# lh3/ropebwt2

Measured on AMD Instinct MI355X. Metric: Gsymbols/s inserted (wall-clock), bit-identical .fmd, higher is better.
Workload: dtype u8; 1 GPU; configs[1]: 100000000 x 101 bp synthetic reads (splitmix64 seed 42), -bsR -m4g, 1 x MI355X; step = one -m batch (40844297/40844297/18311406 reads); 20 steps = 7 job(s) of 3 batches, each job on an empty index (the last job stops after batch 2); reads_per_job=100000000, symbols=69532236588, symbols_per_gpu=69532236588, parallelism=1 GPU, driver=single engine, counts_ok=True

## Files before the change

ropebwt2_amd/csrc/rb2_kernels.h:

```cpp
#pragma once
#include "rb2_device.h"

namespace rb2 {


__device__ __forceinline__ uint32_t zero_bytes(uint32_t x)
{
	const uint32_t t = ((x & 0x7f7f7f7fu) + 0x7f7f7f7fu) | x;
	return __popc(~t & 0x80808080u);
}

__device__ __forceinline__ void load64(const uint8_t *s, uint64_t len, uint64_t base, uint32_t w[16])
{
	if (base + 64 <= len) {
		const uint4 *p = (const uint4*)(s + base);
#pragma unroll
		for (int i = 0; i < 4; ++i) { uint4 v = p[i]; w[4*i] = v.x; w[4*i+1] = v.y; w[4*i+2] = v.z; w[4*i+3] = v.w; }
	} else {
#pragma unroll
		for (int i = 0; i < 16; ++i) {
			uint32_t x = 0;
			for (int k = 0; k < 4; ++k) {
				const uint64_t p = base + 4*i + k;
				x |= (uint32_t)(p < len ? s[p] : 0xffu) << (8*k);
// ... 1185 lines not shown
		const int v = min(GSYM, max(0, (int)nvalid - ln * GSYM));
		pl_acc(A, b0, b1, b2, bits_below((uint32_t)v));
		uint64_t *dst = (uint64_t*)newp.data + gl * LEAFW + ln;
		dst[0] = b0; dst[LEAFG] = b1; dst[2 * LEAFG] = b2;
	}
	const uint32_t r0 = wave_sum<uint32_t>(A.p0 | A.p1 << 16), r1 = wave_sum<uint32_t>(A.p2 | A.p01 << 16), r2 = wave_sum<uint32_t>(A.p02);
	if (ln == 0) {
		PlAcc T;
		T.p0 = r0 & 0xffffu; T.p1 = r0 >> 16; T.p2 = r1 & 0xffffu; T.p01 = r1 >> 16; T.p02 = r2;
		uint32_t c[6];
		pl_finish(T, nvalid, c);
		LeafMeta m;
		for (int sy = 0; sy < 6; ++sy) m.c[sy] = (uint16_t)c[sy];
		m.npre = 0; m.n = (uint16_t)nvalid;
		newp.own[gl] = m;
	}
	__builtin_amdgcn_fence(__ATOMIC_SEQ_CST, "wavefront"); __builtin_amdgcn_wave_barrier();
	}
}


__device__ __forceinline__ void split_body(Ctl *ctl, const PoolView &pool, const uint32_t *SPL, uint32_t spl_cap, uint32_t epoch , Mailbox *mb,
		const uint32_t bidx, const uint32_t nblk, uint16_t (*s_row)[7][SB], uint32_t round1)
{
	const uint32_t tid = threadIdx.x & 255u;
	if (bidx == 0 && tid == 0) mb->progress = round1;
	if (ctl->overflow) { if (bidx == 0 && tid == 0) mb->void_round = ctl->overflow; return; }
	const int wv = __builtin_amdgcn_readfirstlane(tid >> 6);
	const int ln = lane_id();
	const uint32_t nsp_raw = ctl->nsplit2[(round1 - 1u) & 1u];
	const uint32_t nsp_all = min(nsp_raw, spl_cap);
	if (nsp_raw > spl_cap && bidx == 0 && tid == 0) { ctl->sbfull = 1; mb->respread = 1; }
	for (uint32_t e = bidx * MW + wv; e < nsp_all; e += nblk * MW) {
		const uint64_t gl = SPL[e], sb = gl / SB;
		uint32_t mine = 0;
		if (ln == 0) mine = atomicExch((uint32_t*)dir_row(pool, sb, 7), epoch) != epoch;
		if (!__shfl((int)mine, 0)) continue;
		uint16_t v[7];
#pragma unroll
		for (int r = 0; r < 7; ++r) v[r] = ln < SB ? dir_row(pool, sb, r)[ln] : (uint16_t)0;
		const uint32_t used = (uint32_t)__popcll(__ballot(ln < SB && (v[0] & FILL_MASK) > 0));
		uint32_t marked = (uint32_t)__ballot(ln < SB && (v[0] & FILL_MASK) > (uint32_t)(LEAF - SP_MARGIN));
		if (marked == 0) continue;
		const uint32_t room = SB - used;
		if ((uint32_t)__popc(marked) > room) {
			if (ln == 0) { ctl->sbfull = 1; mb->respread = 1; }
			while ((uint32_t)__popc(marked) > room) marked &= ~(1u << (31 - __builtin_clz(marked)));
			if (marked == 0) continue;
		}
		const uint32_t first = (uint32_t)__builtin_ctz(marked);
		uint16_t (*R)[SB] = s_row[wv];
		if (ln < (int)used && !((marked >> ln) & 1u)) {
			const uint32_t nj = (uint32_t)ln + (uint32_t)__popc(marked & ((1u << ln) - 1u));
#pragma unroll
			for (int r = 0; r < 7; ++r) R[r][nj] = v[r];
		}
		uint64_t *leaves = (uint64_t*)pool.data + sb * SB * LEAFW;
		const bool wl = ln < LEAFW;
		const uint32_t gq = (uint32_t)(ln & 15);
		for (int c0 = SB - 8; c0 >= 0; c0 -= 8) {
		if ((uint32_t)(c0 + 8) <= first || (uint32_t)c0 >= used) continue;
		uint64_t W[8];
#pragma unroll
		for (int j = 0; j < 8; ++j) { const uint32_t k = (uint32_t)(c0 + j); W[j] = (wl && k >= first && k < used) ? leaves[(uint64_t)k * LEAFW + ln] : 0ull; }
#pragma unroll
		for (int j = 0; j < 8; ++j) {
			const int k = c0 + j;
			if ((uint32_t)k < first || (uint32_t)k >= used) continue;
			const uint32_t nk = (uint32_t)k + (uint32_t)__popc(marked & ((1u << k) - 1u));
			const uint64_t w = W[j];
			if (!((marked >> k) & 1u)) { if (nk != (uint32_t)k && wl) leaves[(uint64_t)nk * LEAFW + ln] = w; continue; }
			const uint32_t nraw = (uint32_t)__builtin_amdgcn_readlane((int)v[0], k), n = nraw & FILL_MASK, p2f = nraw & FILL_P2;
			uint32_t ck[6];
#pragma unroll
			for (int s = 0; s < 6; ++s) ck[s] = (uint32_t)__builtin_amdgcn_readlane((int)v[1 + s], k);
			const uint32_t hg = (n / 2) >> 6, h = hg << 6;
			const uint64_t w1 = (uint64_t)__shfl((unsigned long long)w, (ln + 16) & 63), w2 = (uint64_t)__shfl((unsigned long long)w, (ln + 32) & 63);
			PlAcc A;
			pl_acc(A, w, w1, leaf_p2(p2f != 0, w, w1, w2), (ln < LEAFG && gq < hg) ? ~0ull : 0ull);
			const uint32_t r0 = lane63(dpp_incl_add(A.p0 | A.p1 << 16)), r1 = lane63(dpp_incl_add(A.p2 | A.p01 << 16)), r2 = lane63(dpp_incl_add(A.p02));
			PlAcc T;
			T.p0 = r0 & 0xffffu; T.p1 = r0 >> 16; T.p2 = r1 & 0xffffu; T.p01 = r1 >> 16; T.p02 = r2;
			uint32_t c1[6];
			pl_finish(T, h, c1);
			const uint64_t up = (uint64_t)__shfl((unsigned long long)w, (ln + (int)hg) & 63);
			if (wl) {
				leaves[(uint64_t)(nk + 1) * LEAFW + ln] = gq + hg < (uint32_t)LEAFG ? up : 0ull;
				leaves[(uint64_t)nk * LEAFW + ln] = gq < hg ? w : 0ull;
			}
			if (ln == 0) {
				R[0][nk] = (uint16_t)(h | p2f); R[0][nk + 1] = (uint16_t)((n - h) | p2f);
#pragma unroll
				for (int s = 0; s < 6; ++s) { R[1 + s][nk] = (uint16_t)c1[s]; R[1 + s][nk + 1] = (uint16_t)(ck[s] - c1[s]); }
			}
		}
		}
		__builtin_amdgcn_fence(__ATOMIC_SEQ_CST, "wavefront"); __builtin_amdgcn_wave_barrier();
		const uint32_t nused = used + (uint32_t)__popc(marked);
		if (ln == 0) atomicAdd((unsigned long long*)&ctl->nsplit_total, (unsigned long long)__popc(marked));
		if ((uint32_t)ln >= first && (uint32_t)ln < nused) {
#pragma unroll
			for (int r = 0; r < 7; ++r) dir_row(pool, sb, r)[ln] = R[r][ln];
		}
		__builtin_amdgcn_fence(__ATOMIC_SEQ_CST, "wavefront"); __builtin_amdgcn_wave_barrier();
	}
}
__global__ __launch_bounds__(256) void k_split(Ctl *ctl, PoolView pool, const uint32_t *SPL, uint32_t spl_cap, uint32_t epoch, Mailbox *mb, SbBase *scan2, uint32_t round1)
{
	__shared__ uint16_t s_row[MW][7][SB];
	const uint32_t nb = gridDim.x - (scan2 ? 1u : 0u);
	if (scan2 && blockIdx.x == nb) { __shared__ uint64_t s_w2[4]; sbscan2_lean<256, 2>(ctl, scan2, s_w2); return; }
	split_body(ctl, pool, SPL, spl_cap, epoch, mb, blockIdx.x, nb, s_row, round1);
}

}
#include "rb2_merge.h"
namespace rb2 {


template <bool STRIDE> __global__ __launch_bounds__(256) void k_meta_sb(const Ctl *ctl, int nside, PoolView newp, SbTot *sbtot, int sparse)
{
	const int ln = lane_id();
	const uint64_t nsb = ctl->nsb_total;
	for (uint64_t sbw = ((uint64_t)blockIdx.x * 4 + wave_id()) * 2; sbw < nsb; sbw += (uint64_t)gridDim.x * 8) {
	const uint64_t sb = sbw + (ln >> 5);
	const bool live = sb < nsb;
	const uint64_t gl = sb * SB + (ln & 31);
	const uint64_t sb0 = ctl->rope[nside][ln < NR ? ln : NR - 1].sb0;
	const uint64_t sbA = sb - (ln >> 5);
	const int rA = max(0, (int)__popcll(__ballot(ln < NR && sb0 <= sbA)) - 1);
	const int rB = max(0, (int)__popcll(__ballot(ln < NR && sb0 <= sbA + 1)) - 1);
	const RopeDesc &rp = ctl->rope[nside][(ln >> 5) ? rB : rA];
	const bool ok = live && gl >= rp.leaf0 && gl < rp.leaf0 + rp.nleaves;
	LeafMeta m;
	for (int s = 0; s < 6; ++s) m.c[s] = 0;
	m.npre = 0; m.n = 0;
	if (ok) m = newp.own[gl];
	const uint32_t e01 = m.c[0] | (uint32_t)m.c[1] << 16, e23 = m.c[2] | (uint32_t)m.c[3] << 16, e45 = m.c[4] | (uint32_t)m.c[5] << 16;
	uint32_t s01 = dpp_incl_add(e01), s23 = dpp_incl_add(e23), s45 = dpp_incl_add(e45);
	const uint32_t h01 = (uint32_t)__builtin_amdgcn_readlane((int)s01, 31), h23 = (uint32_t)__builtin_amdgcn_readlane((int)s23, 31), h45 = (uint32_t)__builtin_amdgcn_readlane((int)s45, 31);
	if (ln >> 5) { s01 -= h01; s23 -= h23; s45 -= h45; }
	const uint32_t x01 = s01 - e01, x23 = s23 - e23, x45 = s45 - e45;
	if (sparse) {
		if (live) {
			uint16_t *dr = dir_row(newp, sb, 0) + (ln & 31);
			dr[0] = (uint16_t)(m.n | ((m.c[0] | m.c[5]) ? FILL_P2 : 0u));
#pragma unroll
			for (int s = 0; s < 6; ++s) dr[(1 + s) * SB] = m.c[s];
			dr[7 * SB] = 0;
		}
	} else if (ok) {
		m.c[0] = (uint16_t)x01; m.c[1] = (uint16_t)(x01 >> 16); m.c[2] = (uint16_t)x23; m.c[3] = (uint16_t)(x23 >> 16);
		m.c[4] = (uint16_t)x45; m.c[5] = (uint16_t)(x45 >> 16);
		m.npre = (uint16_t)((x01 & 0xffffu) + (x01 >> 16) + (x23 & 0xffffu) + (x23 >> 16) + (x45 & 0xffffu) + (x45 >> 16));
		newp.meta[gl] = m;
	}
	if ((ln & 31) == 31 && live) {
		SbTot c;
		c.p01 = s01; c.p23 = s23; c.p45 = s45; c.pad = 0;
		sbtot[sb] = c;
	}
	if (!STRIDE) return;
	}
}

constexpr int SBT = 4;
constexpr int SB2T = 512;
template <int NT, int CT = 8> __device__ __forceinline__ void sbscan2_body(const Ctl *ctl, SbBase *base, uint64_t (*s_w)[NT / 64])
{
	constexpr int SB2T = NT;
	const uint64_t nc = (ctl->nsb_total + SCHUNK - 1) / SCHUNK;
	const int ln = lane_id(), wv = __builtin_amdgcn_readfirstlane(threadIdx.x >> 6);
	uint64_t run[6] = {0, 0, 0, 0, 0, 0};
	for (uint64_t i0 = 0; i0 < nc; i0 += CT * SB2T) {
		const uint64_t j0 = i0 + (uint64_t)threadIdx.x * CT;
		uint64_t v[CT][6], tot[6] = {0, 0, 0, 0, 0, 0};
#pragma unroll
		for (int k = 0; k < CT; ++k)
#pragma unroll
			for (int s = 0; s < 6; ++s) v[k][s] = j0 + k < nc ? base[j0 + k].cum[s] : 0ull;
#pragma unroll
		for (int k = 0; k < CT; ++k)
#pragma unroll
			for (int s = 0; s < 6; ++s) { const uint64_t x = v[k][s]; v[k][s] = tot[s]; tot[s] += x; }
		uint64_t inc[6];
#pragma unroll
		for (int s = 0; s < 6; ++s) { inc[s] = wave_incl_add<uint64_t>(tot[s]); if (ln == 63) s_w[s][wv] = inc[s]; }
		__syncthreads();
		uint64_t b0[6];
#pragma unroll
		for (int s = 0; s < 6; ++s) {
			uint64_t off = 0, all = 0;
			for (int w = 0; w < SB2T / 64; ++w) { const uint64_t x = s_w[s][w]; if (w < wv) off += x; all += x; }
			b0[s] = run[s] + off + inc[s] - tot[s];
			run[s] += all;
		}
#pragma unroll
		for (int k = 0; k < CT; ++k) if (j0 + k < nc) {
			SbBase o;
#pragma unroll
			for (int s = 0; s < 6; ++s) o.cum[s] = b0[s] + v[k][s];
			o.pos = o.cum[0] + o.cum[1] + o.cum[2] + o.cum[3] + o.cum[4] + o.cum[5]; o.pad = 0;
			base[j0 + k] = o;
		}
		__syncthreads();
	}
	if (threadIdx.x == 0) {
		SbBase o;
#pragma unroll
		for (int s = 0; s < 6; ++s) o.cum[s] = run[s];
		o.pos = run[0] + run[1] + run[2] + run[3] + run[4] + run[5]; o.pad = 0;
		base[nc] = o;
	}
}
template <int NT, int CT> __device__ __forceinline__ void sbscan2_col(const Ctl *ctl, SbBase *base, uint64_t *s_w, const int col)
{
	const uint64_t nc = (ctl->nsb_total + SCHUNK - 1) / SCHUNK;
	const int ln = lane_id(), wv = __builtin_amdgcn_readfirstlane(threadIdx.x >> 6);
	uint64_t *colp = col < 6 ? &base[0].cum[col] : &base[0].pos;
	uint64_t run = 0;
#pragma unroll 1
	for (uint64_t i0 = 0; i0 < nc; i0 += (uint64_t)CT * NT) {
		const uint64_t j0 = i0 + (uint64_t)threadIdx.x * CT;
		uint64_t v[CT], tot = 0;
#pragma unroll
		for (int k = 0; k < CT; ++k) v[k] = j0 + k < nc ? colp[(j0 + k) * 8] : 0ull;
#pragma unroll
		for (int k = 0; k < CT; ++k) { const uint64_t x = v[k]; v[k] = tot; tot += x; }
		const uint64_t inc = dpp_incl_add64(tot);
		if (ln == 63) s_w[wv] = inc;
		__syncthreads();
		uint64_t off = 0, all = 0;
		for (int w = 0; w < NT / 64; ++w) { const uint64_t x = s_w[w]; if (w < wv) off += x; all += x; }
		const uint64_t b0 = run + off + inc - tot;
#pragma unroll
		for (int k = 0; k < CT; ++k) if (j0 + k < nc) colp[(j0 + k) * 8] = b0 + v[k];
		run += all;
		__syncthreads();
	}
	if (threadIdx.x == 0) { colp[nc * 8] = run; if (col == 6) base[nc].pad = 0; }
}
static_assert(sizeof(SbBase) == 64, "sbscan2_col strides over the records in 64-bit words");
template <int NT, int CT> __device__ __forceinline__ void sbscan2_lean(const Ctl *ctl, SbBase *base, uint64_t *s_w)
{
#pragma unroll 1
	for (int col = 0; col < 7; ++col) sbscan2_col<NT, CT>(ctl, base, s_w, col);
}
__global__ __launch_bounds__(SB2T) void k_sbscan2(const Ctl *ctl, SbBase *base)
{
	__shared__ uint64_t s_w[6][SB2T / 64];
	sbscan2_body<SB2T>(ctl, base, s_w);
}
__device__ __forceinline__ void sbscan3_body(const Ctl *ctl, const SbTot *sbtot, const PoolView &newp, const uint32_t blk, uint32_t (*s_p)[4])
{
	const uint64_t n = ctl->nsb_total, i0 = (uint64_t)blk * SCHUNK + (uint64_t)threadIdx.x * SBT;
	if ((uint64_t)blk * SCHUNK >= n) return;
	const int ln = lane_id(), wv = __builtin_amdgcn_readfirstlane(threadIdx.x >> 6);
	uint32_t e[SBT][6], tot[6] = {0, 0, 0, 0, 0, 0}, own[SBT];
#pragma unroll
	for (int k = 0; k < SBT; ++k) {
		SbTot t; t.p01 = t.p23 = t.p45 = t.pad = 0;
		if (i0 + k < n) t = sbtot[i0 + k];
		const uint32_t v[6] = { t.p01 & 0xffffu, t.p01 >> 16, t.p23 & 0xffffu, t.p23 >> 16, t.p45 & 0xffffu, t.p45 >> 16 };
		own[k] = v[0] + v[1] + v[2] + v[3] + v[4] + v[5];
#pragma unroll
		for (int s = 0; s < 6; ++s) { e[k][s] = tot[s]; tot[s] += v[s]; }
	}
	uint32_t inc[6];
#pragma unroll
	for (int s = 0; s < 6; ++s) { inc[s] = dpp_incl_add(tot[s]); if (ln == 63) s_p[s][wv] = inc[s]; }
	__syncthreads();
	uint32_t b0[6];
#pragma unroll
	for (int s = 0; s < 6; ++s) {
		uint32_t off = 0;
#pragma unroll
		for (int w = 0; w < 3; ++w) if (w < wv) off += s_p[s][w];
		b0[s] = off + inc[s] - tot[s];
	}
	if (threadIdx.x < 6) newp.sbbase[blk].cum[threadIdx.x] = (uint64_t)s_p[threadIdx.x][0] + s_p[threadIdx.x][1] + s_p[threadIdx.x][2] + s_p[threadIdx.x][3];
	if (threadIdx.x == 6) {
		uint64_t p = 0;
#pragma unroll
		for (int s = 0; s < 6; ++s) p += (uint64_t)s_p[s][0] + s_p[s][1] + s_p[s][2] + s_p[s][3];
		newp.sbbase[blk].pos = p;
	}
#pragma unroll
	for (int k = 0; k < SBT; ++k) if (i0 + k < n) {
		uint32_t o[6];
#pragma unroll
		for (int s = 0; s < 6; ++s) o[s] = b0[s] + e[k][s];
		uint4 *q = (uint4*)&newp.sbrec[i0 + k];
		q[0] = make_uint4(o[0], o[1], o[2], o[3]);
		q[1] = make_uint4(o[4], o[5], o[0] + o[1] + o[2] + o[3] + o[4] + o[5], own[k]);
	}
}
__global__ __launch_bounds__(SCHUNK / SBT) void k_sbscan3(const Ctl *ctl, const SbTot *sbtot, PoolView newp)
{
	__shared__ uint32_t s_p[6][4];
	sbscan3_body(ctl, sbtot, newp, blockIdx.x, s_p);
}


template <bool AE, bool SPARSE, typename P> __device__ __forceinline__ bool advance_tile(const uint32_t tile, const Ctl *ctl, int side, int is_comp, uint32_t round, const uint8_t *s, const PoolView &newp,
		const StrArrays<P> &S, ShardRec *send, const PushTab *push)
{
	const P *L = S.L, *SIZE = S.SIZE, *INS_E = S.INS_E, *RKOLD = S.RKOLD; const uint64_t *W = S.W; const uint8_t *A = S.A; const TileFix *tf = S.tf; const uint16_t *RKREL = S.RKREL;
	P *L2 = S.L2, *U2 = S.U2; uint64_t *W2 = S.W2; uint8_t *A2 = S.A2;
	__shared__ GroupLds G;
	const TileFix &tfx = tf[tile];
	const SegDesc &sg = ctl->seg[side];
	if ((ctl->ne[round & 1] == 0) != AE) return false;
	if (SPARSE && ctl->overflow) return false;
	if (tile >= sg.tile0[NR]) return false;
	TileCtx t;
	tile_ctx_fix(tfx, t);
	int sym2[2], flag2[2];
	uint64_t w2[2]; P l2[2];
	uint32_t araw[2];
	const uint32_t fixw = tilefix_word(tf, tile);
	const uint32_t nval = (uint32_t)min((uint64_t)STILE, t.segend - t.base);
	{
		const uint64_t *Wb = W + t.base; const P *Lb = L + t.base; const uint8_t *Ab = A + t.base;
#pragma unroll
		for (int h = 0; h < 2; ++h) {
			const uint32_t x = (uint32_t)(h * 256) + threadIdx.x;
			w2[h] = 0; l2[h] = 0; araw[h] = 7;
			if (x < nval) { w2[h] = Wb[x]; l2[h] = Lb[x]; araw[h] = Ab[x]; }
		}
	}
	__shared__ P s_acb[6]; __shared__ uint32_t s_dst[6];
	const RopeDesc &nrp = ctl->rope[side ^ 1][t.b];
	__shared__ uint32_t s_pr[6];
	if (threadIdx.x < 6) {
		const int a6 = threadIdx.x;
		s_acb[a6] = SPARSE ? (P)ctl->ac[t.b][a6] : (P)(ctl->ac[t.b][a6] - sb_cum(newp, nrp.sb0, a6));
		s_dst[a6] = (uint32_t)(push ? ctl->pdst[t.b][a6] : ctl->dest[t.b][a6]);
		s_pr[a6] = push ? ctl->pdev[t.b][a6] : 0u;
	}
	const int orda[6] = { sym_ord(0, is_comp), sym_ord(1, is_comp), sym_ord(2, is_comp), sym_ord(3, is_comp), sym_ord(4, is_comp), sym_ord(5, is_comp) };
	P rk[2], sz[2]; uint64_t wv[2];
	bool act0[2];
	struct RankRaw { P sbb; uint32_t sbr, meta, rkrel; };
	const uint64_t sb0u = uniform64(nrp.sb0), leaf0u = uniform64(nrp.leaf0);
	const LeafMeta *metab = newp.meta + leaf0u; const SbRec *sbrb = newp.sbrec + sb0u;
	const uint16_t *RKb = RKREL + t.segstart; const P *Eb = INS_E + t.segstart; const P *ROb = SPARSE ? RKOLD + t.segstart : nullptr;
	auto rank_issue = [&](int h, int a, uint32_t slot, P F, bool flag, RankRaw &q) {
		if (SPARSE) {
			q.sbb = ROb[slot]; q.sbr = 0; q.meta = 0; q.rkrel = RKb[slot];
			return;
		}
		const P f = (P)(((!AE && flag) ? Eb[slot] : (P)(l2[h] - F)) + (P)slot);
		const uint32_t lf = (uint32_t)(f >> LEAF_SH), sbq = (uint32_t)sb0u + lf / SB;
		if (sizeof(P) == 4) {
			const uint32_t ua = (uint32_t)a;
			q.sbb = *(const P*)((const char*)newp.sbbase + ((sbq >> SCHUNK_SH) * (uint32_t)sizeof(SbBase) + ua * 8u));
			q.sbr = *(const uint32_t*)((const char*)sbrb + ((lf / SB) * (uint32_t)sizeof(SbRec) + ua * 4u));
			q.meta = *(const uint16_t*)((const char*)metab + (lf * (uint32_t)sizeof(LeafMeta) + ua * 2u));
			q.rkrel = *(const uint16_t*)((const char*)RKb + slot * 2u);
			return;
		}
		const P *bb = (const P*)&newp.sbbase[sbq >> SCHUNK_SH].cum[a];
		q.sbb = *bb; q.sbr = sbrb[lf / SB].cum[a]; q.meta = metab[lf].c[a]; q.rkrel = RKb[slot];
	};
	auto rank_sum = [](const RankRaw &q) -> P { return (P)(q.sbb + q.sbr + q.meta + q.rkrel); };
	RankRaw rq[2];
	const bool spec = (tfx.nexthead & 4u) != 0;
#pragma unroll
	for (int h = 0; h < 2; ++h) {
		const uint32_t x = (uint32_t)(h * 256) + threadIdx.x;
		const int a = (int)(araw[h] & 7u);
		act0[h] = (uint32_t)(a - 1) < 6u;
		RB2_UNDEFV(rq[h].sbb); RB2_UNDEFV(rq[h].sbr); RB2_UNDEFV(rq[h].meta); RB2_UNDEFV(rq[h].rkrel);
		const uint32_t slot = (uint32_t)t.lt * STILE + x;
		if (spec && act0[h]) rank_issue(h, a, slot, (P)slot, (araw[h] & 0x40u) != 0, rq[h]);
	}
	uint32_t rt[2][4]; bool need[2], fastr[2];
	const uint64_t tlen = ctl->len;
#pragma unroll
	for (int h = 0; h < 2; ++h) {
		sz[h] = 0;
		wv[h] = cur_next(w2[h]);
		need[h] = act0[h] && cur_empty(wv[h]);
		const uint64_t tp = cur_pos(wv[h]);
		fastr[h] = need[h] && tp + 16 <= tlen;
		const uint32_t *q = fastr[h] ? (const uint32_t*)(s + (tp & ~3ull)) : (const uint32_t*)ctl;
		rt[h][0] = q[0]; rt[h][1] = q[1]; rt[h][2] = q[2]; rt[h][3] = q[3];
	}
	group_setup(G, t, araw, fixw, sym2, flag2);
	uint32_t nz = 0;
	bool act[2];
	Member mem[2];
#pragma unroll
	for (int h = 0; h < 2; ++h) {
		const int x = h * 256 + threadIdx.x;
		act[h] = (uint32_t)x < nval && sym2[h] != 0;
		if (act[h]) mem[h] = group_member(G, t, x, sym2[h], orda);
	}
	if (!spec || !G.allsingle) {
#pragma unroll
		for (int h = 0; h < 2; ++h) if (act[h]) rank_issue(h, sym2[h], mem[h].slot, (P)mem[h].F, flag2[h] != 0, rq[h]);
	}
#pragma unroll
	for (int h = 0; h < 2; ++h) {
		rk[h] = rank_sum(rq[h]);
		if (need[h]) {
			const uint64_t tp = cur_pos(wv[h]);
			wv[h] = fastr[h] ? cur_make(tp + CUR_SYMS, pack9_words(rt[h][0], rt[h][1], rt[h][2], rt[h][3], (uint32_t)(tp & 3) * 8)) : cur_refill(s, tlen, wv[h]);
		}
	}
	if (!AE) {
#pragma unroll
		for (int h = 0; h < 2; ++h) if (act[h] && flag2[h]) sz[h] = (SIZE + t.base)[(uint32_t)(h * 256) + threadIdx.x];
	}
#pragma unroll
	for (int h = 0; h < 2; ++h) {
		if (!act[h]) continue;
		const int a = sym2[h];
		const Member &m = mem[h];
		const P l = SPARSE ? (P)(s_acb[a] + rk[h] + (P)m.pga)
		                   : (P)(s_acb[a] + rk[h] - (P)m.pa + (P)m.pga);
		const P u = (P)(l + sz[h]);
		const uint32_t d = s_dst[a] + m.pa;
		if (push) {
			const uint32_t pr = s_pr[a];
			push->L2[pr][d] = l; push->W2[pr][d] = wv[h]; push->A2[pr][d] = (uint8_t)cur_sym(wv[h]);
			push->U2[pr][d] = u;
			if (!AE && u != l) push->ctl[pr]->ne[(round & 1) ^ 1] = 1;
		} else if (send) {
			send[ctl->sdest[t.b][a] + m.pa] = shard_pack((uint64_t)l, (uint64_t)(u - l), 0u, wv[h]);
		} else {
			L2[d] = l; W2[d] = wv[h]; A2[d] = (uint8_t)cur_sym(wv[h]);
			if (!AE) { U2[d] = u; nz += (u != l); }
		}
	}
	if (!AE && !send && !push) {
		if (__any(nz != 0) && lane_id() == 0) ((Ctl*)ctl)->ne[(round & 1) ^ 1] = 1;
	}
	return true;
}

struct ScanRide { const SbTot *sbtot; uint32_t nscan; };

template <bool AE, bool SPARSE = false, bool STRIDE = false, typename P = uint64_t> __global__ __launch_bounds__(256) void k_advance(const Ctl *ctl, int side, int is_comp, uint32_t round, const uint8_t *s, PoolView newp,
		StrArrays<P> S, ShardRec *send, const PushTab *push, ScanRide sr)
{
	uint32_t nsc = 0;
	if (SPARSE) {
		nsc = sr.nscan;
		if (blockIdx.x < nsc) { __shared__ uint32_t s_p[6][4]; sbscan3_body(ctl, sr.sbtot, newp, blockIdx.x, s_p); return; }
	}
	for (uint32_t tile = (SPARSE && nsc) ? blockIdx.x - nsc : (STRIDE ? blockIdx.x : xcd_item()); ; ) {
		if (!advance_tile<AE, SPARSE, P>(tile, ctl, side, is_comp, round, s, newp, S, send, push)) return;
		if (!STRIDE) return;
		tile += gridDim.x - nsc;
		if (tile >= ctl->seg[side].tile0[NR]) return;
		__syncthreads();
	}
}


__device__ __forceinline__ uint64_t splitmix(uint64_t seed, uint64_t k)
{
	uint64_t z = seed + (k + 1) * 0x9E3779B97F4A7C15ull;
	z = (z ^ (z >> 30)) * 0xBF58476D1CE4E5B9ull;
	z = (z ^ (z >> 27)) * 0x94D049BB133111EBull;
	return z ^ (z >> 31);
}

constexpr uint64_t COV_SALT = 0x5bd1e995c0f3a1d7ull;
__device__ __forceinline__ uint64_t synth_base_index(uint64_t i, uint32_t j, uint32_t L, uint64_t seed, uint64_t genome_len)
{
	return genome_len ? splitmix(seed ^ COV_SALT, i) % (genome_len - L + 1) + j : i * L + j;
}
__device__ __forceinline__ uint32_t synth_base(uint64_t z, int skew)
{
	if (!skew) return (uint32_t)(z >> 62);
	const uint32_t u = (uint32_t)(z >> 56);
	return u < 218u ? 0u : 1u + (u - 218u) % 3u;
}
__device__ __forceinline__ uint8_t synth_byte(uint64_t g, uint64_t first, uint64_t per, uint32_t L, uint64_t seed, uint64_t genome_len, int skew)
{
	const uint64_t r = g / per; uint32_t off = (uint32_t)(g % per);
	const uint64_t i = first + r;
	if (off < L) return (uint8_t)(1 + synth_base(splitmix(seed, synth_base_index(i, L - 1 - off, L, seed, genome_len)), skew));
	if (off == L) return 0;
	off -= L + 1;
	return off < L ? (uint8_t)(4 - synth_base(splitmix(seed, synth_base_index(i, off, L, seed, genome_len)), skew)) : 0;
}
__global__ __launch_bounds__(256) void k_synth(uint8_t *dst, uint64_t first, uint64_t n_reads, uint32_t L, uint64_t seed, int strand, uint64_t genome_len, int skew)
{
	const uint64_t per = (uint64_t)(L + 1) * (strand ? 2 : 1), total = n_reads * per;
	const uint64_t g0 = ((uint64_t)blockIdx.x * 256 + threadIdx.x) * 16;
	if (g0 >= total) return;
	if (g0 + 16 <= total) {
		uint32_t w[4] = {0, 0, 0, 0};
#pragma unroll
		for (int k = 0; k < 16; ++k) w[k >> 2] |= (uint32_t)synth_byte(g0 + k, first, per, L, seed, genome_len, skew) << ((k & 3) * 8);
		*(uint4*)(dst + g0) = make_uint4(w[0], w[1], w[2], w[3]);
	} else for (uint64_t g = g0; g < total; ++g) dst[g] = synth_byte(g, first, per, L, seed, genome_len, skew);
}

__global__ __launch_bounds__(256) void k_rank_batch(const Ctl *ctl, int side, PoolView pv, int b, const uint64_t *x, uint64_t n, uint64_t *out, int sparse)
{
	const uint64_t i = (uint64_t)blockIdx.x * MW + (threadIdx.x >> 6);
	if (i >= n) return;
	uint64_t p = x[i], acc[6] = {0, 0, 0, 0, 0, 0};
	for (int r = 0; r < NR && p > 0; ++r) {
		if (rope_sym(r) != b) continue;
		const RopeDesc &d = ctl->rope[side][r];
		uint64_t c[6];
		if (p >= d.n) { for (int s = 0; s < 6; ++s) acc[s] += d.cnt[s]; p -= d.n; continue; }
		if (sparse) wave_rank_all<true>(pv, d, p, c); else wave_rank_all<false>(pv, d, p, c);
		for (int s = 0; s < 6; ++s) acc[s] += c[s];
		p = 0;
	}
	if (lane_id() < 6) { uint64_t v = acc[0]; for (int s = 1; s < 6; ++s) if (lane_id() == s) v = acc[s]; out[i * 6 + lane_id()] = v; }
}

__global__ __launch_bounds__(256) void k_piece_hash(const Ctl *ctl, int side, PoolView pv, int r, unsigned long long *out)
{
	__shared__ uint64_t s_w[4];
	const RopeDesc &d = ctl->rope[side][r];
	const uint64_t ng = (d.n + GSYM - 1) / GSYM;
	const uint64_t *w = (const uint64_t*)pv.data + d.leaf0 * LEAFW;
	uint64_t acc = 0;
	for (uint64_t j = (uint64_t)blockIdx.x * 256 + threadIdx.x; j < 3 * ng; j += (uint64_t)gridDim.x * 256) {
		const uint64_t G = j / 3; const uint32_t pl = (uint32_t)(j - 3 * G);
		uint64_t v = w[(G >> 4) * LEAFW + pl * LEAFG + (G & 15)];
		if (G == ng - 1) v &= bits_below((uint32_t)(d.n - G * GSYM));
		acc += v * (2 * j + 1);
	}
	uint64_t tot;
	block_excl_add<uint64_t>(acc, s_w, &tot);
	if (threadIdx.x == 0 && tot) atomicAdd(out, (unsigned long long)tot);
}

__global__ __launch_bounds__(64) void k_rank_piece(const Ctl *ctl, int side, PoolView pv, int r, uint64_t p, uint64_t *out, int sparse)
{
	const RopeDesc &d = ctl->rope[side][r];
	uint64_t c[6];
	if (sparse) wave_rank_all<true>(pv, d, p, c); else wave_rank_all<false>(pv, d, p, c);
	if (lane_id() < 6) { uint64_t v = c[0]; for (int s = 1; s < 6; ++s) if (lane_id() == s) v = c[s]; out[lane_id()] = v; }
}

constexpr int LDT = 32;
constexpr int LDB = 256 * LDT;
constexpr uint32_t LD_LONG = 4096;
struct LdPieces {
	uint64_t q[7];
	uint64_t word0[6];
	uint32_t keep[6];
	int32_t  r[6];
	int32_t  np, pad;
};
struct LdLong { uint64_t word0, o, n; uint32_t c, pad; };

__device__ __forceinline__ int ld_dec43(const uint8_t *p, const uint8_t *end, uint32_t &c, uint64_t &l)
{
	const uint32_t b0 = p[0];
	c = b0 & 7u;
	if ((b0 & 0x80u) == 0) { l = b0 >> 3; return 1; }
	if ((b0 >> 5) == 6u) { if (p + 2 > end) return 0; l = ((uint64_t)(b0 & 0x18u) << 3) | (p[1] & 0x3fu); return 2; }
	const int nb = (b0 & 0x10u) ? 8 : 4;
	if (p + nb > end) return 0;
	uint64_t v = (b0 >> 3) & 1u;
	for (int i = 1; i < nb; ++i) v = (v << 6) | (p[i] & 0x3fu);
	l = v;
	return nb;
}
template <typename F> __device__ __forceinline__ void ld_runs(const uint8_t *rle, uint64_t nbytes, uint64_t o0, uint32_t *bad, F f)
{
	const uint64_t o1 = min(o0 + LDT, nbytes);
	for (uint64_t i = o0; i < o1; ++i) {
		if ((rle[i] & 0xc0u) == 0x80u) continue;
		uint32_t c; uint64_t l;
		const int nb = ld_dec43(rle + i, rle + nbytes, c, l);
		if (nb == 0 || c > 5u) { *bad = 1; continue; }
		f(c, l);
	}
}

__global__ __launch_bounds__(256) void k_ld_count(const uint8_t *rle, uint64_t nbytes, uint64_t *blk_n, unsigned long long *tot6, uint32_t *bad)
{
	__shared__ uint64_t s_w[4];
	__shared__ unsigned long long s_c[6];
	if (threadIdx.x < 6) s_c[threadIdx.x] = 0;
	__syncthreads();
	uint64_t n = 0, cnt[6] = {0, 0, 0, 0, 0, 0};
	ld_runs(rle, nbytes, ((uint64_t)blockIdx.x * 256 + threadIdx.x) * LDT, bad, [&](uint32_t c, uint64_t l) {
		n += l;
#pragma unroll
		for (int s = 0; s < 6; ++s) cnt[s] += c == (uint32_t)s ? l : 0ull;
	});
#pragma unroll
	for (int c = 0; c < 6; ++c) { const uint64_t w = wave_sum<uint64_t>(cnt[c]); if (lane_id() == 0 && w) atomicAdd(&s_c[c], (unsigned long long)w); }
	uint64_t tot;
	block_excl_add<uint64_t>(n, s_w, &tot);
	if (threadIdx.x == 0) blk_n[blockIdx.x] = tot;
	if (threadIdx.x < 6 && s_c[threadIdx.x]) atomicAdd(&tot6[threadIdx.x], s_c[threadIdx.x]);
}

__global__ __launch_bounds__(256) void k_ld_expand(const uint8_t *rle, uint64_t nbytes, const uint64_t *blk_off, LdPieces tab_arg, uint64_t *data,
		unsigned long long *pcnt , LdLong *longs, uint32_t *nlong, uint32_t long_cap, uint32_t *bad)
{
	__shared__ uint64_t s_w[4];
	__shared__ unsigned long long s_pc[6][6];
	__shared__ LdPieces tab;
	if (threadIdx.x == 0) tab = tab_arg;
	if (threadIdx.x < 36) s_pc[threadIdx.x / 6][threadIdx.x % 6] = 0;
	const uint64_t o0 = ((uint64_t)blockIdx.x * 256 + threadIdx.x) * LDT;
	uint64_t n = 0;
	ld_runs(rle, nbytes, o0, bad, [&](uint32_t, uint64_t l) { n += l; });
	uint64_t S = blk_off[blockIdx.x] + block_excl_add<uint64_t>(n, s_w, (uint64_t*)0);
	int x = 0;
	uint64_t lc[6] = {0, 0, 0, 0, 0, 0};
	auto tally_out = [&]() {
#pragma unroll
		for (int s = 0; s < 6; ++s) { if (lc[s]) atomicAdd(&s_pc[x][s], (unsigned long long)lc[s]); lc[s] = 0; }
	};
	uint64_t cur_g = ~0ull, cur_w0 = 0, cur_v[3] = {0, 0, 0};
	auto flush = [&]() {
		if (cur_g != ~0ull) {
			unsigned long long *q = (unsigned long long*)&data[cur_w0 + (cur_g >> 4) * LEAFW + (cur_g & 15)];
#pragma unroll
			for (int pl = 0; pl < 3; ++pl) if (cur_v[pl]) atomicOr(q + pl * LEAFG, (unsigned long long)cur_v[pl]);
		}
		cur_v[0] = cur_v[1] = cur_v[2] = 0;
	};
	ld_runs(rle, nbytes, o0, bad, [&](uint32_t c, uint64_t l) {
		while (l > 0) {
			if (x < tab.np && S >= tab.q[x + 1]) { tally_out(); while (x < tab.np && S >= tab.q[x + 1]) ++x; }
			if (x >= tab.np) { *bad = 2; return; }
			const uint64_t part = min(l, tab.q[x + 1] - S), o = S - tab.q[x];
#pragma unroll
			for (int s = 0; s < 6; ++s) lc[s] += c == (uint32_t)s ? part : 0ull;
			if (tab.keep[x] && c != 0) {
				if (part > LD_LONG) {
					const uint32_t k = atomicAdd(nlong, 1u);
					if (k < long_cap) { LdLong e; e.word0 = tab.word0[x]; e.o = o; e.n = part; e.c = c; e.pad = 0; longs[k] = e; }
				} else {
					uint64_t gd = o >> 6; uint32_t off = (uint32_t)(o & 63), t = (uint32_t)part;
					while (t > 0) {
						const uint32_t k = min(t, (uint32_t)GSYM - off);
						const uint64_t field = bits_below(k) << off;
						if (gd != cur_g || tab.word0[x] != cur_w0) { flush(); cur_g = gd; cur_w0 = tab.word0[x]; }
						if (c & 1u) cur_v[0] |= field;
						if (c & 2u) cur_v[1] |= field;
						if (c & 4u) cur_v[2] |= field;
						t -= k; off = 0; ++gd;
					}
				}
			}
			S += part; l -= part;
		}
	});
	flush();
	if (x < tab.np) tally_out();
	__syncthreads();
	if (threadIdx.x < 36) {
		const int px = threadIdx.x / 6, c = threadIdx.x % 6;
		if (px < tab.np && s_pc[px][c]) atomicAdd(&pcnt[tab.r[px] * 6 + c], s_pc[px][c]);
	}
}

__global__ __launch_bounds__(256) void k_ld_long(const LdLong *longs, const uint32_t *nlong, uint32_t long_cap, uint64_t *data)
{
	const uint32_t n = min(*nlong, long_cap);
	for (uint32_t e = blockIdx.x; e < n; e += gridDim.x) {
		const LdLong L = longs[e];
		const uint64_t g0 = L.o >> 6, g1 = (L.o + L.n - 1) >> 6;
		for (uint64_t gd = g0 + threadIdx.x; gd <= g1; gd += 256) {
			const uint64_t lo = max(L.o, gd << 6), hi = min(L.o + L.n, (gd + 1) << 6);
			const uint64_t field = bits_below((uint32_t)(hi - lo)) << (uint32_t)(lo & 63);
			unsigned long long *q = (unsigned long long*)&data[L.word0 + (gd >> 4) * LEAFW + (gd & 15)];
#pragma unroll
			for (int pl = 0; pl < 3; ++pl) if ((L.c >> pl) & 1u) atomicOr(q + pl * LEAFG, (unsigned long long)field);
		}
	}
}

__global__ __launch_bounds__(256) void k_ld_own(PoolView pv, uint64_t leaf0, uint64_t nleaves, uint64_t n)
{
	const uint64_t i = (uint64_t)blockIdx.x * MW + wave_id();
	if (i >= nleaves) return;
	const uint32_t fill = (uint32_t)min((uint64_t)LEAF, n - i * LEAF);
	uint32_t c[6];
	wave_leaf_counts(leaf_words(pv.data, leaf0 + i), 0, fill, c);
	if (lane_id() == 0) {
		LeafMeta m;
		for (int s = 0; s < 6; ++s) m.c[s] = (uint16_t)c[s];
		m.npre = 0; m.n = (uint16_t)fill;
		pv.own[leaf0 + i] = m;
	}
}

}
```

Before: 23.08 Gsymbols/s.

## Stage advance-tile outputs in LDS for coalesced per-symbol global writes

In the non-sparse, non-send, non-push path, each thread now writes its computed l, w and u values into shared-memory buffers ordered by symbol run, instead of scattering them straight to global memory. After a block barrier, threads read those buffers back contiguously and write L2/W2/A2/U2 so that consecutive threads store to consecutive destinations. The goal is to replace scattered global stores with coalesced ones. The cost is extra LDS use (which may lower occupancy), a __syncthreads, and a compiler memory barrier.

New measurement: 23.35 Gsymbols/s (median of 6 runs). +1.2%, better.

```diff
diff --git a/ropebwt2_amd/csrc/rb2_kernels.h b/ropebwt2_amd/csrc/rb2_kernels.h
--- a/ropebwt2_amd/csrc/rb2_kernels.h
+++ b/ropebwt2_amd/csrc/rb2_kernels.h
@@ -1511,6 +1511,9 @@
 }
 
 
+#ifndef RB2_ADV_STAGE
+#define RB2_ADV_STAGE 1
+#endif
 template <bool AE, bool SPARSE, typename P> __device__ __forceinline__ bool advance_tile(const uint32_t tile, const Ctl *ctl, int side, int is_comp, uint32_t round, const uint8_t *s, const PoolView &newp,
 		const StrArrays<P> &S, ShardRec *send, const PushTab *push)
 {
@@ -1598,6 +1601,14 @@
 	}
 	group_setup(G, t, araw, fixw, sym2, flag2);
 	uint32_t nz = 0;
+	constexpr bool STAGED = RB2_ADV_STAGE != 0 && !SPARSE;
+	__shared__ uint64_t s_sw[STAGED ? STILE : 1]; __shared__ P s_sl[STAGED ? STILE : 1], s_su[STAGED && !AE ? STILE : 1];
+	const bool stage = STAGED && !send && !push;
+	auto run_starts = [&](uint32_t rs[7]) {
+		rs[0] = rs[1] = 0;
+#pragma unroll
+		for (int a6 = 1; a6 < 6; ++a6) rs[a6 + 1] = rs[a6] + G.cpre[8][a6];
+	};
 	bool act[2];
 	Member mem[2];
 #pragma unroll
@@ -1622,6 +1633,7 @@
 #pragma unroll
 		for (int h = 0; h < 2; ++h) if (act[h] && flag2[h]) sz[h] = (SIZE + t.base)[(uint32_t)(h * 256) + threadIdx.x];
 	}
+	if (STAGED) asm volatile("" ::: "memory");
 #pragma unroll
 	for (int h = 0; h < 2; ++h) {
 		if (!act[h]) continue;
@@ -1638,9 +1650,34 @@
 			if (!AE && u != l) push->ctl[pr]->ne[(round & 1) ^ 1] = 1;
 		} else if (send) {
 			send[ctl->sdest[t.b][a] + m.pa] = shard_pack((uint64_t)l, (uint64_t)(u - l), 0u, wv[h]);
+		} else if (stage) {
+			uint32_t rs[7], r = 0;
+			run_starts(rs);
+#pragma unroll
+			for (int a6 = 2; a6 < 6; ++a6) r = a == a6 ? rs[a6] : r;
+			const uint32_t j = r + (m.pa - G.fix.tpre[a]);
+			s_sl[j] = l; s_sw[j] = wv[h];
+			if (!AE) { s_su[j] = u; nz += (u != l); }
 		} else {
 			L2[d] = l; W2[d] = wv[h]; A2[d] = (uint8_t)cur_sym(wv[h]);
 			if (!AE) { U2[d] = u; nz += (u != l); }
+		}
+	}
+	if (stage) {
+		__syncthreads();
+		uint32_t rs[7];
+		run_starts(rs);
+#pragma unroll
+		for (int h = 0; h < 2; ++h) {
+			const uint32_t j = (uint32_t)(h * 256) + threadIdx.x;
+			if (j >= rs[6]) continue;
+			int a = 1; uint32_t r = 0;
+#pragma unroll
+			for (int a6 = 2; a6 < 6; ++a6) if (j >= rs[a6]) { a = a6; r = rs[a6]; }
+			const uint32_t d = s_dst[a] + G.fix.tpre[a] + (j - r);
+			const uint64_t wj = s_sw[j];
+			L2[d] = s_sl[j]; W2[d] = wj; A2[d] = (uint8_t)cur_sym(wj);
+			if (!AE) U2[d] = s_su[j];
 		}
 	}
 	if (!AE && !send && !push) {
```
